# ucla-vision/xivo

Measured on AMD Instinct MI355X. Metric: EKF updates/sec (state dim 250, 80 feats) @1 GPU; % MFMA roofline, higher is better.
Workload: dtype f64; 1 GPU; MH gating + UpdateJosephForm: state dim 250, 80 features (M=160), XIVO row sparsity, P/H/inn/R resident in HBM; filters_per_gpu=16384, global_batch=16384, parallelism=replicas x1 (no collective), pipeline=sparse-H (row-pair compressed H, whitened in-solve Joseph form), hand_over=dense H -> row-pair compressed rows every step, inside the timed region, route=sparse_in_solve, not_spd_filters=0

## Files before the change

### xivo_amd/csrc/capi_update.hip

```cpp
#include <algorithm>

#include "capi_internal.h"

using namespace xivo_hip;
using namespace xivo_hip::capi;

namespace {

enum UpdateRoute : int { ROUTE_FUSED = 0, ROUTE_SPARSE_IN_SOLVE, ROUTE_SPARSE_WHITENED, ROUTE_SPARSE_SYMMETRIC, ROUTE_SPARSE_TAIL,
                         ROUTE_DENSE_ASCODED, ROUTE_DENSE_WHITENED, ROUTE_DENSE_SYMMETRIC, ROUTE_COUNT };
static const char* kRouteNames[ROUTE_COUNT] = {"fused", "sparse_in_solve", "sparse_whitened", "sparse_symmetric", "sparse_tail",
                                               "dense_ascoded", "dense_whitened", "dense_symmetric"};
struct UpdatePlan {
  int route;
  bool sparse;
  bool in_solve;
  bool latency;
  bool stream8;
  bool f32_whitened;
};

static UpdatePlan plan_update(const xivo_hip_ctx* c, int b0, int B, bool gate) {
  const StagedRows& r = c->rows;
  const int Np = c->Np, Mp = r.rows_padded();
// ... 106 lines not shown
    StageTimer st(c, ST_TRSM, (2.0 * Mf * Mf * Nf + 32.0 * Mf * Nf + (plan.in_solve ? 2.0 * t_outs_f * Mf : 0.0)) * B, label,
                  8.0 * B * (0.5 * Mp * (Mp + 1) + Mp / 16 * 512.0 + (plan.in_solve ? 1.0 : 3.0) * Np * Mp + (plan.in_solve ? t_outs + (double)Np * Np : 0.0)));
    HIP_TRY((hipError_t)(narrow ? launch_trsm_narrow(a, c->stream) : launch_trsm_f64(a, c->stream)));
    if (plan.in_solve) return XIVO_HIP_OK;
  }
  GemmExtra x; x.epi = EPI_RSUB_MAT; x.msub = v.P; x.lower_only = 1; x.skip = v.status;
  x.small_tiles = plan.latency;
  if (plan.f32_whitened) {
    x.fp32 = 1; x.a_f32 = 1; x.b_f32 = 1;
    const WhitenedF32 w = whitened_f32(v.G, Np, Mp);
    return gemm(c, ST_PNEW, B, Np, Np, {w.V, w.Y, Mp}, v.P, x);
  }
  return gemm(c, ST_PNEW, B, Np, Np, {v.K, v.G, Mp}, v.P, x);
}

static int update_sparse_range(xivo_hip_ctx* c, const UpdatePlan& plan, const UpdateViews& v, int b0, int B, const UpdateGate* gate) {
  const int Np = c->Np, Mp = c->rows.rows_padded();
  const BatchMat &P = v.P, &HP = v.HP, &PHT = v.PHT, &S = v.S, &K = v.K, &G = v.G, &T = v.T;
  const BatchVec &inn = v.inn, &diagR = v.diagR;
  const EllBuffers& e = v.ell;
  const auto [nc_max, pw_max] = c->rows.max_slots(b0, B);
  const double Nf = c->N, Mf = c->rows.rows();
  const double nnz_flops = 2.0 * Mf * 21.0;
  int rc;
  if (plan.route == ROUTE_FUSED) {
    FusedArgs a{};
    P.to(a.P, a.strideP, a.ldp); a.ell = e; inn.to(a.inn, a.strideInn); diagR.to(a.diagR, a.strideR);
    v.err.to(a.err, a.strideErr); PHT.to(a.PHT, a.stridePHT, a.ldpht); a.status = v.status;
    a.Np = Np; a.Mp = Mp; a.batch = B; a.pw = pw_max;
    if (gate) {
      a.gate = 1; a.F = gate->F; a.gp = gate->gp;
      a.mask = c->mask + (long)b0 * gate->F; a.dist = c->dist + (long)b0 * gate->F;
      if (c->rows.dense_alive()) { v.H.to(a.H, a.strideH, a.ldh); v.HT.to(a.HT, a.strideHT, a.ldht); }
    }
    char label[64]; fused_update_label(Mp, Np, pw_max, label, sizeof(label));
    const double t_outs_f = 0.5 * Nf * (Nf + 1.0);
    StageTimer st(c, ST_TRSM, (nnz_flops * (Nf + Mf) + Mf * Mf * Mf / 3.0 + 2.0 * Mf * Mf * Nf + 32.0 * Mf * Nf + 2.0 * t_outs_f * Mf) * B, label,
                  B * (16.0 * Np * Np + (Mp / 2) * ELL_W * 20.0));
    HIP_TRY((hipError_t)launch_fused_update(a, c->stream));
    return XIVO_HIP_OK;
  }
  const int mr0 = c->rows.mixed_row0();
  const int Mp_ell = mr0 >= 0 ? round_up16(mr0) : Mp;
  const int oos_pad = mr0 >= 0 ? round_up16(Mp - mr0) : 0;
  bool walk_tiled = false;
  const int oos_k = (mr0 >= 0 && c->have_layout) ? std::min(Np, round_up16(c->lay.group_begin + 6 * c->lay.n_groups)) : Np;
  {
    EllMulArgs a{}; a.ell = e; P.to(a.Src, a.strideSrc, a.ldsrc); PHT.to(a.out, a.strideOut, a.ldo);
    HP.to(a.out2, a.strideOut2, a.ldo2); a.X = Np; a.Mp = Mp_ell; a.batch = B; a.nc_max = nc_max; a.pw_max = pw_max; a.cols = Np;
    char label[64]; ell_kernel_label(ELL_HP, a, label, sizeof(label));
    walk_tiled = ell_uses_slab_form(a);
    StageTimer st(c, ST_HP, nnz_flops * Nf * B, label, 8.0 * B * ((double)Np * Np + (double)Np * Mp));
    HIP_TRY((hipError_t)launch_ell_mul(ELL_HP, a, c->stream));
  }
  if (mr0 >= 0) {
    GemmExtra x; x.C2 = PHT.at(0, mr0);
    rc = gemm(c, ST_HP, B, oos_pad, Np, {v.H.at(mr0, 0), P, oos_k}, HP.at(mr0, 0), x);
    if (rc) return rc;
  }
  const bool lead = c->rows.has_lead() && mr0 < 0;
  if (lead) {
    GemmExtra x; x.epi = EPI_ADD_MAT; x.msub = PHT; x.C2 = HP;
    x.c2_rows = walk_tiled ? LEAD_K : 0;
    rc = gemm(c, ST_HP, B, Np, Mp, {P, v.lead, LEAD_K}, PHT, x);
    if (rc) return rc;
  }
  GateEllArgs ga{};
  if (gate) {
    ga.ell = e;
    v.H.to(ga.H, ga.strideH, ga.ldh); v.HT.to(ga.HT, ga.strideHT, ga.ldht);
    if (!c->rows.dense_alive()) { ga.H = nullptr; ga.HT = nullptr; }
    ga.PHT = PHT.p;
    inn.to(ga.inn, ga.strideInn); diagR.to(ga.diagR, ga.strideR);
    ga.mask = c->mask + (long)b0 * gate->F; ga.dist = c->dist + (long)b0 * gate->F;
    ga.F = gate->F; ga.Np = Np; ga.batch = B;
    S.to(ga.S, ga.strideS, ga.lds); ga.Mp = Mp; ga.gp = gate->gp;
  }
  const BatchVec Sdiag{T.p, T.stride};
  int diag_done = 0;
  {
    EllMulArgs a{}; a.ell = e; PHT.to(a.Src, a.strideSrc, a.ldsrc); HP.to(a.SrcAlt, a.strideSrcAlt, a.ldsrcAlt);
    S.to(a.out, a.strideOut, a.ldo); a.cols = Np;
    diagR.to(a.diagR, a.strideR); a.X = Mp; a.Mp = Mp_ell; a.batch = B; a.nc_max = nc_max; a.pw_max = pw_max;
    if (gate && mr0 < 0 && !lead && (long)2 * Mp <= Sdiag.stride) { Sdiag.to(a.diag_out, a.strideDiag); a.diag_done = &diag_done; }
    char label[64]; ell_kernel_label(ELL_S, a, label, sizeof(label));
    StageTimer st(c, ST_S, nnz_flops * Mf * B, label, 8.0 * B * ((double)Np * Mp + (double)Mp * Mp));
    HIP_TRY((hipError_t)launch_ell_mul(ELL_S, a, c->stream));
  }
  if (mr0 >= 0) {
    GemmExtra x; x.epi = EPI_ADD_DIAG; x.diag = BatchVec{diagR.p + mr0, diagR.stride}; x.lower_only = 1;
    rc = gemm(c, ST_S, B, oos_pad, oos_pad, {HP.at(mr0, 0), v.H.at(mr0, 0), oos_k}, S.at(mr0, mr0), x);
    if (rc) return rc;
  }
  if (lead) {
    GemmExtra x; x.epi = EPI_ADD_MAT; x.msub = S; x.lower_only = 1;
    rc = gemm(c, ST_S, B, Mp, Mp, {HP, v.lead, LEAD_K}, S, x);
    if (rc) return rc;
  }
  CholGateArgs cg{};
  bool gate_folded = false;
  if (gate) {
    if (diag_done) Sdiag.to(ga.Sdiag, ga.strideSdiag);
    gate_folded = diag_done && !c->rows.dense_alive() && mr0 < 0 && !plan.latency && chol_gate_supported(Mp, B);
    if (gate_folded) {
      Sdiag.to(cg.Sdiag, cg.strideSdiag); inn.to(cg.inn, cg.strideInn); diagR.to(cg.diagR, cg.strideR);
      cg.ellval = e.val; cg.strideVal = e.stride_val(); cg.ell_w = ELL_W; PHT.to(cg.PHT, cg.stridePHT, cg.ldpht); cg.Np = Np;
      cg.mask = ga.mask; cg.dist = ga.dist; cg.F = gate->F; cg.gp = gate->gp;
    } else {
      StageTimer st(c, ST_GATE, 0.0, "gate_ell_kernel");
      HIP_TRY((hipError_t)launch_gate_ell(ga, c->stream));
    }
  }
  if (plan.route != ROUTE_SPARSE_TAIL && plan.route != ROUTE_SPARSE_SYMMETRIC)
    return finish_whitened(c, plan, v, B, gate_folded ? &cg : nullptr);
  rc = factor_S(c, v, B, 0, gate_folded ? &cg : nullptr, Mf * Mf * Mf / 3.0 * B);
  if (rc) return rc;
  if (plan.route == ROUTE_SPARSE_SYMMETRIC) return finish_symmetric(c, plan, v, B);
  const bool t_here = trsm_forms_T(Mp, Np);
  {
    TrsmArgs a = trsm_args(c, v, B);
    if (t_here) { T.to(a.T, a.strideT, a.ldt); P.to(a.Pm, a.stridePm, a.ldpm); }
    char label[64]; trsm_kernel_label(Mp, label, sizeof(label), t_here ? 1 : 0);
    const double t_outs = 0.5 * Np * (Np + 1.0), t_outs_f = 0.5 * Nf * (Nf + 1.0);
    StageTimer st(c, ST_TRSM, (2.0 * Mf * Mf * Nf + (t_here ? 2.0 * t_outs_f * Mf : 0.0)) * B, label,
                  8.0 * B * (0.5 * Mp * (Mp + 1) + Mp / 16 * 512.0 + 2.0 * Np * Mp + (t_here ? t_outs + (double)Np * Np : 0.0)));
    HIP_TRY((hipError_t)launch_trsm_f64(a, c->stream));
  }
  if (!t_here) {
    GemmExtra x; x.epi = EPI_SUB_MAT; x.msub = P; x.lower_only = 1;
    rc = gemm(c, ST_AP, B, Np, Np, {K, PHT, Mp}, T, x);
    if (rc) return rc;
  }
  {
    EllMulArgs a{}; a.ell = e; T.to(a.Src, a.strideSrc, a.ldsrc); G.to(a.out, a.strideOut, a.ldo);
    diagR.to(a.diagR, a.strideR); K.to(a.K, a.strideK, a.ldk); a.X = Np; a.Mp = Mp; a.batch = B; a.nc_max = nc_max; a.pw_max = pw_max; a.cols = Np;
    char label[64]; ell_kernel_label(ELL_G, a, label, sizeof(label));
    StageTimer st(c, ST_KH, nnz_flops * Np * B, label, 8.0 * B * ((double)Np * Np + 2.0 * Np * Mp));
    HIP_TRY((hipError_t)launch_ell_mul(ELL_G, a, c->stream));
  }
  if (pnew_reg_supported(Mp, Np)) {
    PnewRegArgs a{}; G.to(a.G, a.strideG, a.ldg); K.to(a.K, a.strideK, a.ldk);
    T.to(a.T, a.strideT, a.ldt); P.to(a.P, a.strideP, a.ldp);
    a.skip_status = v.status; a.Mp = Mp; a.Np = Np; a.batch = B;
    char label[64]; pnew_reg_kernel_label(Mp, label, sizeof(label));
    const double outs = 0.5 * Np * (Np + 1.0);
    StageTimer st(c, ST_PNEW, 2.0 * outs * Mp * B, label, 8.0 * B * (2.0 * Np * Mp + outs + (double)Np * Np));
    HIP_TRY((hipError_t)launch_pnew_reg_f64(a, c->stream));
    return XIVO_HIP_OK;
  }
  GemmExtra x; x.epi = EPI_SUB_MAT; x.msub = T; x.lower_only = 1;
  x.skip = v.status;
  return gemm(c, ST_PNEW, B, Np, Np, {G, K, Mp}, P, x);
}

static int update_dense_range(xivo_hip_ctx* c, const UpdatePlan& plan, const UpdateViews& v, int b0, int B, const UpdateGate* gate) {
  const int Np = c->Np, Mp = c->rows.rows_padded();
  const BatchMat &H = v.H, &HT = v.HT, &P = v.P, &HP = v.HP, &PHT = v.PHT, &S = v.S, &K = v.K, &A = v.KHI, &T = v.T;
  int rc = ensure_dense(c);
  if (rc) return rc;
  {
    GemmExtra x; x.C2 = PHT;
    rc = gemm(c, ST_HP, B, Mp, Np, {H, P, Np}, HP, x);
    if (rc) return rc;
  }
  if (gate) {
    rc = ensure_HT(c);
    if (rc) return rc;
    GateDenseArgs a{};
    H.to(a.Hw, a.strideH, a.ldh); HT.to(a.HTw, a.strideHT, a.ldht);
// ... 417 lines not shown
```

### xivo_amd/csrc/ell.h

```cpp
#pragma once
#include "common.h"

namespace xivo_hip {

constexpr int ELL_CW = 16, ELL_PW = 12, ELL_W = ELL_CW + ELL_PW;
constexpr int ELL_PIW = 12;

struct EllBuffers {
  int* idx;
  double* val;
  int* nc;
  int* pw;
  int* over;
  int pairs_max;
  __host__ __device__ long stride_idx() const { return (long)pairs_max * ELL_W; }
  __host__ __device__ long stride_val() const { return (long)pairs_max * ELL_W * 2; }
};

int launch_meas_compress(const double* H, long strideH, int ldh, const double* inn, long strideInn,
                         const double* diagR, long strideR, int M, int N, int Np, int Mp_clear, EllBuffers e,
                         double* inn_out, long strideInnOut, double* R_out, long strideROut, int batch, hipStream_t s,
                         int* host_flags = nullptr );
bool meas_compress_fits(int Mp_clear, int Np);
int launch_meas_vectors(const double* inn, long strideInn, const double* diagR, long strideR, int M, int Mp_clear, EllBuffers e,
                        double* inn_out, long strideInnOut, double* R_out, long strideROut, int batch, hipStream_t s);
int launch_ell_to_dense(EllBuffers e, double* H, long strideH, int ldh, double* HT, long strideHT, int ldht, int Mp,
                        int Np, int batch, hipStream_t s, int Mrows = -1);
int launch_zero_rows(double* H, long strideH, int ldh, int row0, int nrows, int c0, int c1, int batch, hipStream_t s);

enum EllMode : int {
  ELL_HP = 0,
  ELL_S = 1,
  ELL_G = 2,
  ELL_GF = 3,
};
struct GateEllArgs {
  EllBuffers ell;
  double* H; long strideH; int ldh;
  double* HT; long strideHT; int ldht;
  double* PHT;
  double* inn; long strideInn;
  double* diagR; long strideR;
  unsigned char* mask; double* dist;
  int F, Np, batch;
  GateParams gp;
  double* S; long strideS; int lds; int Mp;
  const double* Sdiag; long strideSdiag;
};
struct EllMulArgs {
  EllBuffers ell;
  const double* Src; long strideSrc; int ldsrc;
  int cols;
  const double* SrcAlt; long strideSrcAlt; int ldsrcAlt;
  double* out; long strideOut; int ldo;
  double* out2; long strideOut2; int ldo2;
  double* diag_out; long strideDiag;
  int* diag_done;
  const double* diagR; long strideR;
  const double* K; long strideK; int ldk;
  int X;
  int Mp;
  int slabs_per_wg;
  int persist_stride;
  int rb_per_wg;
  int nc_max;
  int pw_max;
  int batch;
};
int launch_ell_mul(int mode, const EllMulArgs& a, hipStream_t s);
void ell_kernel_label(int mode, const EllMulArgs& a, char* buf, size_t n);
bool ell_uses_slab_form(const EllMulArgs& a);

int launch_gate_ell(const GateEllArgs& a, hipStream_t s);

}
```

### xivo_amd/csrc/ell_kernels.hip

```cpp
#include "ell.h"
#include <stdio.h>
#include <stdlib.h>

namespace xivo_hip {

namespace {

struct MeasCompressArgs {
  const double* H; long strideH; int ldh;
  const double* inn; long strideInn;
  const double* diagR; long strideR;
  int M, N, Np;
  int pairs_clear;
  EllBuffers ell;
  double* inn_out; long strideInnOut;
  double* R_out; long strideROut;
  int list_ld;
  int* host_flags;
};

template <bool ALIGNED, int UNR = 16>
__global__ __launch_bounds__(256) void meas_compress_kernel(MeasCompressArgs a) {
  extern __shared__ __attribute__((aligned(16))) double csh[];
  const int filt = blockIdx.x, tid = threadIdx.x, lane = tid & 63, wave = tid >> 6, nw = blockDim.x >> 6;
// ... 152 lines not shown
__global__ __launch_bounds__(256) void zero_rows_kernel(double* Hall, long strideH, int ldh, int row0, int nrows, int c0, int c1) {
  double* H = Hall + (long)blockIdx.x * strideH;
  for (long i = threadIdx.x; i < (long)nrows * (c1 - c0); i += 256) H[row0 + (i % nrows) + (long)(c0 + i / nrows) * ldh] = 0.0;
}

template <int MODE, int CWU>
__global__ __launch_bounds__(256) void ell_mul_kernel(EllMulArgs a) {
  const int xchunks = (a.X + 255) / 256;
  const int nrb = a.Mp / 16;
  const int rsplit = (nrb + a.rb_per_wg - 1) / a.rb_per_wg;
  const int per = rsplit * xchunks;
  const int b = blockIdx.x;
  const int xcd = b & 7, slot = b >> 3;
  const int filt = (slot / per) * 8 + xcd;
  if (filt >= a.batch) return;
  const int sub = slot % per;
  const int rs = sub / xchunks, xc = sub % xchunks;
  const int x = xc * 256 + threadIdx.x;
  const bool live = x < a.X;
  const int xs = live ? x : 0;
  const double* __restrict__ Src = a.Src + (long)filt * a.strideSrc + xs;
  const int* __restrict__ idx0 = a.ell.idx + (long)filt * a.ell.stride_idx();
  const double* __restrict__ val0 = a.ell.val + (long)filt * a.ell.stride_val();

  double cm[CWU];
#pragma unroll
  for (int t = 0; t < CWU; ++t) cm[t] = Src[(long)idx0[t] * a.ldsrc];

  const double* __restrict__ dR = a.diagR + (long)filt * a.strideR;
  const double* __restrict__ K = a.K + (long)filt * a.strideK + xs;
  double* __restrict__ out = a.out + (long)filt * a.strideOut + xs;
  double* __restrict__ out2 = a.out2 + (long)filt * a.strideOut2 + (long)xs * a.ldo2;
  const int p_end = 8 * min(nrb, (rs + 1) * a.rb_per_wg);
#pragma unroll 2
  for (int p = 8 * rs * a.rb_per_wg; p < p_end; ++p) {
    const int* __restrict__ pi = idx0 + (long)p * ELL_W + ELL_CW;
    const double* __restrict__ pv = val0 + (long)p * ELL_W * 2;
    double sv[ELL_PW];
#pragma unroll
    for (int t = 0; t < ELL_PW; ++t) sv[t] = Src[(long)pi[t] * a.ldsrc];
    double a0 = 0.0, a1 = 0.0;
#pragma unroll
    for (int t = 0; t < CWU; ++t) { a0 = fma(pv[2 * t], cm[t], a0); a1 = fma(pv[2 * t + 1], cm[t], a1); }
#pragma unroll
    for (int t = 0; t < ELL_PW; ++t) {
      a0 = fma(pv[2 * (ELL_CW + t)], sv[t], a0); a1 = fma(pv[2 * (ELL_CW + t) + 1], sv[t], a1);
    }
    if (!live) continue;
    const int m = 2 * p;
    if (MODE == ELL_HP) {
      out[(long)m * a.ldo] = a0;
      out[(long)(m + 1) * a.ldo] = a1;
      *reinterpret_cast<d2*>(out2 + m) = d2{a0, a1};
    } else if (MODE == ELL_S) {
      out[(long)m * a.ldo] = a0 + (x == m ? dR[m] : 0.0);
      out[(long)(m + 1) * a.ldo] = a1 + (x == m + 1 ? dR[m + 1] : 0.0);
    } else {
      out[(long)m * a.ldo] = fma(K[(long)m * a.ldk], dR[m], a0);
      out[(long)(m + 1) * a.ldo] = fma(K[(long)(m + 1) * a.ldk], dR[m + 1], a1);
    }
  }
}

typedef __attribute__((address_space(4))) const double ell_cdouble;
typedef __attribute__((address_space(4))) const int ell_cint;

constexpr bool ell_tile_pf(int mode, int cwu, int xc, int pwu) {
  return xc == 64 && cwu == 12 && mode == ELL_S && pwu >= 0;
}
typedef unsigned ell_u2 __attribute__((ext_vector_type(2)));
__device__ __forceinline__ __amdgpu_buffer_rsrc_t ell_rsrc(const void* p) {
  return __builtin_amdgcn_make_buffer_rsrc(const_cast<void*>(p), 0, 0x7FFFFFFF, 0x00020000);
}
__device__ __forceinline__ double ell_buf_ld(__amdgpu_buffer_rsrc_t r, unsigned voff, unsigned soff) {
  return __builtin_bit_cast(double, __builtin_amdgcn_raw_buffer_load_b64(r, voff, soff, 0));
}
__device__ __forceinline__ void ell_buf_st(double v, __amdgpu_buffer_rsrc_t r, unsigned voff, unsigned soff) {
  __builtin_amdgcn_raw_buffer_store_b64(__builtin_bit_cast(ell_u2, v), r, voff, soff, 0);
}

constexpr bool ell_tile_mf(int mode, int cwu, int xc, int pwu) {
  return (xc == 64 || xc == 32) && cwu % 4 == 0 && pwu % 3 == 0 && (mode == ELL_HP || mode == ELL_S);
}
constexpr int ell_tile_threads(int mode, int cwu, int xc, int pwu) {
  return (mode == ELL_S || ell_tile_pf(mode, cwu, xc, pwu)) ? 512 : 1024;
}

template <int MODE, int CWU, int XC, int PWU, bool TALL = true>
__global__ __launch_bounds__(ell_tile_threads(MODE, CWU, XC, PWU)) void ell_tile_kernel(EllMulArgs a) {
  constexpr int NSLOT = CWU + PWU;
  constexpr int NT = ell_tile_threads(MODE, CWU, XC, PWU), NW = NT / 64;
  constexpr bool PF = ell_tile_pf(MODE, CWU, XC, PWU);
  constexpr int UNR = (PF || (CWU == 12 && XC == 64)) ? 2 : 1;
  constexpr int RN = PF ? (MODE == ELL_S ? (TALL ? 40 : 32) : 34) : 8;
  extern __shared__ __attribute__((aligned(16))) double tile[];
  const int xchunks = (a.X + XC - 1) / XC;
  const int wgs = (xchunks + a.slabs_per_wg - 1) / a.slabs_per_wg;
  const int b = blockIdx.x;
  const int xcd = b & 7, slot = b >> 3;
  int filt = (slot / wgs) * 8 + xcd;
  if (filt >= a.batch) return;
  const int s_begin = (slot % wgs) * a.slabs_per_wg;
  const int s_end = min(xchunks, s_begin + a.slabs_per_wg);
  const int tid = threadIdx.x, lane = tid & 63, wave = __builtin_amdgcn_readfirstlane(tid >> 6);
  const double* Src = a.Src + (long)filt * a.strideSrc;
  const int cols = a.cols;
  const int pairs = a.Mp / 2;
  double* ops = tile + (long)cols * XC;
  unsigned short* pidx = reinterpret_cast<unsigned short*>(ops + (long)pairs * NSLOT * 2);
  auto stage_ops = [&](int f) {
    const d2* __restrict__ gv = reinterpret_cast<const d2*>(a.ell.val + (long)f * a.ell.stride_val());
    for (int e = tid; e < pairs * NSLOT; e += NT) {
      const int p = e / NSLOT, t = e % NSLOT;
      *reinterpret_cast<d2*>(ops + 2 * e) = gv[p * ELL_W + (t < CWU ? t : ELL_CW + (t - CWU))];
    }
    const int* __restrict__ gi = a.ell.idx + (long)f * a.ell.stride_idx();
    for (int e = tid; e < pairs * ELL_PIW; e += NT) {
      const int p = e / ELL_PIW, t = e % ELL_PIW;
      pidx[e] = t < PWU ? (unsigned short)gi[p * ELL_W + ELL_CW + t] : (unsigned short)0;
    }
    if (tid < ELL_CW) pidx[pairs * ELL_PIW + tid] = (unsigned short)gi[tid];
  };
  stage_ops(filt);
  double r[RN];
  auto fetch = [&](const double* FSrc, int sidx) {
    const int x0 = sidx * XC;
    if (MODE == ELL_S) {
      constexpr int KU = RN / (XC / NW);
      const __amdgpu_buffer_rsrc_t rs = ell_rsrc(FSrc);
      const unsigned vo = (unsigned)lane * 8u;
#pragma unroll
      for (int q = 0; q < XC / NW; ++q) {
        const int jj = wave + NW * q;
        const bool ok = x0 + jj < a.X;
        const unsigned so = (unsigned)((x0 + (ok ? jj : 0)) * a.ldsrc) * 8u;
#pragma unroll
        for (int u = 0; u < KU; ++u) {
          const int k = lane + 64 * u;
          r[q * KU + u] = (ok && k < cols) ? ell_buf_ld(rs, vo, so + (unsigned)(64 * u) * 8u) : 0.0;
        }
      }
    } else {
      const int xx = tid % XC, kq = tid / XC;
      const bool ok = x0 + xx < a.X;
      const unsigned voff = ((unsigned)(ok ? xx : 0) + (unsigned)kq * (unsigned)a.ldsrc) * 8u;
      const char* base = reinterpret_cast<const char*>(FSrc + x0);
      const size_t step = (size_t)(NT / XC) * (size_t)a.ldsrc * 8u;
      const int nu = cols / (NT / XC);
#pragma unroll
      for (int u = 0; u < RN; ++u) {
        double v = 0.0;
        if (u < nu) v = *reinterpret_cast<const double*>(base + (size_t)u * step + voff);
        r[u] = ok ? v : 0.0;
      }
    }
  };
  auto park = [&]() {
    if (MODE == ELL_S) {
      constexpr int KU = RN / (XC / NW);
#pragma unroll
      for (int q = 0; q < XC / NW; ++q) {
        const int jj = wave + NW * q;
#pragma unroll
        for (int u = 0; u < KU; ++u) { const int k = lane + 64 * u; if (k < cols) tile[k * XC + (jj ^ (k & 15))] = r[q * KU + u]; }
      }
    } else {
      const int xx = tid % XC, kq = tid / XC;
#pragma unroll
      for (int u = 0; u < RN; ++u) { const int k = kq + (NT / XC) * u; if (k < cols) tile[k * XC + (xx ^ (k & 15))] = r[u]; }
    }
  };

  const int xx = lane % XC, half = lane / XC;
  auto slab = [&](int k) -> double { return tile[k * XC + (xx ^ (k & 15))]; };

  const int fstep = PF ? a.persist_stride : 0;
  if (PF) fetch(Src, s_begin);
  for (;;) {
  ell_cint* idx0 = (ell_cint*)(a.ell.idx + (long)filt * a.ell.stride_idx());
  ell_cdouble* dR = (ell_cdouble*)(a.diagR + (long)filt * a.strideR);
  const int nfilt = filt + fstep;
  const bool more = fstep > 0 && nfilt < a.batch;
  for (int sidx = s_begin; sidx < s_end; ++sidx) {
    if (PF) {
      park();
    } else if (MODE == ELL_S) {
      const int x0 = sidx * XC;
      for (int jj = wave; jj < XC; jj += NW) {
        const bool ok = x0 + jj < a.X;
        const double* __restrict__ col = Src + (long)(x0 + (ok ? jj : 0)) * a.ldsrc;
        for (int k0 = 0; k0 < cols; k0 += 64 * 8) {
#pragma unroll
          for (int u = 0; u < 8; ++u) { const int k = k0 + lane + 64 * u; r[u] = (ok && k < cols) ? col[k] : 0.0; }
#pragma unroll
          for (int u = 0; u < 8; ++u) { const int k = k0 + lane + 64 * u; if (k < cols) tile[k * XC + (jj ^ (k & 15))] = r[u]; }
        }
      }
    } else {
      const int x0 = sidx * XC;
      const int xq = tid % XC, kq = tid / XC;
      const bool ok = x0 + xq < a.X;
      const double* __restrict__ row = Src + x0 + (ok ? xq : 0);
      for (int k0 = 0; k0 < cols; k0 += (NT / XC) * 8) {
#pragma unroll
        for (int u = 0; u < 8; ++u) { const int k = k0 + kq + (NT / XC) * u; r[u] = (ok && k < cols) ? row[(long)k * a.ldsrc] : 0.0; }
#pragma unroll
        for (int u = 0; u < 8; ++u) { const int k = k0 + kq + (NT / XC) * u; if (k < cols) tile[k * XC + (xq ^ (k & 15))] = r[u]; }
      }
    }
    if (PF) asm volatile("s_waitcnt lgkmcnt(0)\n\ts_barrier" ::: "memory");
    else __syncthreads();
    if (PF) {
      if (sidx + 1 < s_end) fetch(Src, sidx + 1);
      else if (more) fetch(a.Src + (long)nfilt * a.strideSrc, s_begin);
    }

    if constexpr (ell_tile_mf(MODE, CWU, XC, PWU)) {
      constexpr int NC = XC / 16, KS = CWU / 4;
      const int li = lane & 15, lg = lane >> 4;
      const unsigned short* cidx = pidx + pairs * ELL_PIW;
      int ck[KS];
#pragma unroll
      for (int s = 0; s < KS; ++s) ck[s] = cidx[4 * s + lg];
      const int x0 = sidx * XC;
      const __amdgpu_buffer_rsrc_t rO = ell_rsrc(a.out + (long)filt * a.strideOut);
      const unsigned vO = (unsigned)(2 * lg * a.ldo + li) * 8u;
      double dRc[NC];
#pragma unroll
      for (int c = 0; c < NC; ++c) dRc[c] = 0.0;
      if (MODE == ELL_S) {
#pragma unroll
        for (int c = 0; c < NC; ++c) if (x0 + 16 * c + li < a.X) dRc[c] = a.diagR[(long)filt * a.strideR + x0 + 16 * c + li];
      }
      const int rb_end = MODE == ELL_S ? min(pairs / 8, NC * (sidx + 1)) : pairs / 8;
      const int pa = (li & 3) + 4 * (li >> 3), ra = (li >> 2) & 1;
      for (int rb = wave; rb < rb_end; rb += NW) {
        const int p0 = 8 * rb;
        d4 acc[NC];
#pragma unroll
        for (int c = 0; c < NC; ++c) acc[c] = d4{0.0, 0.0, 0.0, 0.0};
        if constexpr (NT == 512) {
          uint2 iq[2][ELL_PIW / 4];
  #pragma unroll
          for (int q = 0; q < 2; ++q) {
            const uint2* pq = reinterpret_cast<const uint2*>(pidx + (p0 + lg + 4 * q) * ELL_PIW);
  #pragma unroll
            for (int u = 0; u < ELL_PIW / 4; ++u) iq[q][u] = pq[u];
          }
  #pragma unroll
          for (int q = 0; q < 2; ++q) {
            const int p = p0 + lg + 4 * q;
            const d2* pv = reinterpret_cast<const d2*>(ops) + (long)p * NSLOT + CWU;
            static_assert(PWU % 3 == 0, "three slots per step");
            d2 vn[3];
  #pragma unroll
            for (int u = 0; u < 3; ++u) vn[u] = pv[u];
  #pragma unroll
            for (int t0 = 0; t0 < PWU; t0 += 3) {
              d2 v[3]; double g[3][NC];
  #pragma unroll
              for (int u = 0; u < 3; ++u) {
                const int t = t0 + u;
                v[u] = vn[u];
                const unsigned w = (t & 2) ? iq[q][t >> 2].y : iq[q][t >> 2].x;
                const int k = (int)((t & 1) ? (w >> 16) : (w & 0xffffu));
                const double* trow = tile + k * XC;
                const int sw = k & 15;
  #pragma unroll
                for (int c = 0; c < NC; ++c) g[u][c] = trow[(16 * c + li) ^ sw];
              }
              if (t0 + 3 < PWU) {
  #pragma unroll
                for (int u = 0; u < 3; ++u) vn[u] = pv[t0 + 3 + u];
              }
              __builtin_amdgcn_sched_barrier(0);
  #pragma unroll
              for (int u = 0; u < 3; ++u) {
  #pragma unroll
                for (int c = 0; c < NC; ++c) {
                  acc[c][2 * q] = fma(v[u][0], g[u][c], acc[c][2 * q]);
                  acc[c][2 * q + 1] = fma(v[u][1], g[u][c], acc[c][2 * q + 1]);
                }
              }
            }
          }
        } else {
  #pragma unroll
          for (int q = 0; q < 2; ++q) {
            const int p = p0 + lg + 4 * q;
            const d2* pv = reinterpret_cast<const d2*>(ops) + (long)p * NSLOT + CWU;
            const unsigned short* pkp = pidx + p * ELL_PIW;
            static_assert(PWU % 3 == 0, "three slots per step");
  #pragma unroll 1
            for (int t0 = 0; t0 < PWU; t0 += 3) {
              d2 v[3]; double g[3][NC];
  #pragma unroll
              for (int u = 0; u < 3; ++u) {
                v[u] = pv[t0 + u];
                const int k = (int)pkp[t0 + u];
                const double* trow = tile + k * XC;
                const int sw = k & 15;
  #pragma unroll
                for (int c = 0; c < NC; ++c) g[u][c] = trow[(16 * c + li) ^ sw];
              }
              __builtin_amdgcn_sched_barrier(0);
  #pragma unroll
              for (int u = 0; u < 3; ++u) {
  #pragma unroll
                for (int c = 0; c < NC; ++c) {
                  acc[c][2 * q] = fma(v[u][0], g[u][c], acc[c][2 * q]);
                  acc[c][2 * q + 1] = fma(v[u][1], g[u][c], acc[c][2 * q + 1]);
                }
              }
            }
          }
        }
        {
          double av[KS], cb[KS][NC];
#pragma unroll
          for (int s = 0; s < KS; ++s) {
            av[s] = ops[((long)(p0 + pa) * NSLOT + 4 * s + lg) * 2 + ra];
#pragma unroll
            for (int c = 0; c < NC; ++c) cb[s][c] = tile[ck[s] * XC + ((16 * c + li) ^ (ck[s] & 15))];
          }
#pragma unroll
          for (int c = 0; c < NC; ++c) {
#pragma unroll
            for (int s = 0; s < KS; ++s) acc[c] = __builtin_amdgcn_mfma_f64_16x16x4f64(av[s], cb[s][c], acc[c], 0, 0, 0);
          }
        }
#pragma unroll
        for (int c = 0; c < NC; ++c) {
          const int x = x0 + 16 * c + li;
          if (x >= a.X) continue;
#pragma unroll
          for (int r = 0; r < 4; ++r) {
            const int pp = p0 + lg + 4 * (r >> 1), i = r & 1, m = 2 * pp + i;
            const unsigned sO = (unsigned)((2 * p0 + 8 * (r >> 1) + i) * a.ldo + x0 + 16 * c) * 8u;
            if (MODE == ELL_HP) ell_buf_st(acc[c][r], rO, vO, sO);
            else {
              const double sv_ = acc[c][r] + (x == m ? dRc[c] : 0.0);
              ell_buf_st(sv_, rO, vO, sO);
              if (a.diag_out && (x >> 1) == pp) a.diag_out[(long)filt * a.strideDiag + 4 * pp + 2 * (x & 1) + i] = sv_;
            }
          }
        }
      }
      asm volatile("s_waitcnt lgkmcnt(0)\n\ts_barrier" ::: "memory");
      continue;
    }
    const int x = sidx * XC + xx;
    const bool live = x < a.X;
    const double* __restrict__ K = a.K + (long)filt * a.strideK + (live ? x : 0);
    double* __restrict__ out = a.out + (long)filt * a.strideOut + (live ? x : 0);
    float* __restrict__ outf = reinterpret_cast<float*>(a.out) + (long)filt * a.strideOut + (live ? x : 0);
    double cm[CWU];
#pragma unroll
    for (int t = 0; t < CWU; ++t) cm[t] = slab(idx0[t]);
    const int p_end = MODE == ELL_S ? min(pairs, (sidx * XC + XC) / 2) : pairs;
    double dRx = 0.0;
    if (MODE == ELL_S && live) dRx = a.diagR[(long)filt * a.strideR + x];
#pragma unroll UNR
    for (int p = wave; p < p_end; p += NW) {
      const d2* pv = reinterpret_cast<const d2*>(ops) + (long)p * NSLOT;
      unsigned pk[ELL_PIW];
      {
        const uint2* pq = reinterpret_cast<const uint2*>(pidx + p * ELL_PIW);
#pragma unroll
        for (int u = 0; u < ELL_PIW / 4; ++u) {
          const uint2 q = pq[u];
          pk[4 * u] = q.x & 0xffffu; pk[4 * u + 1] = q.x >> 16; pk[4 * u + 2] = q.y & 0xffffu; pk[4 * u + 3] = q.y >> 16;
        }
      }
      double sv[PWU];
#pragma unroll
      for (int t = 0; t < PWU; ++t) sv[t] = slab((int)pk[t]);
      double a0 = 0.0, a1 = 0.0;
#pragma unroll
      for (int t = 0; t < CWU; ++t) { const d2 v = pv[t]; a0 = fma(v[0], cm[t], a0); a1 = fma(v[1], cm[t], a1); }
#pragma unroll
      for (int t = 0; t < PWU; ++t) { const d2 v = pv[CWU + t]; a0 = fma(v[0], sv[t], a0); a1 = fma(v[1], sv[t], a1); }
      if (!live) continue;
#pragma unroll
      for (int i = 0; i < 2; ++i) {
        if (XC == 32 && i != half) continue;
        const int m = 2 * p + i;
        const double acc = i ? a1 : a0;
        if (MODE == ELL_HP) out[(long)m * a.ldo] = acc;
        else if (MODE == ELL_S) {
          const double sv_ = acc + (x == m ? dRx : 0.0);
          out[(long)m * a.ldo] = sv_;
          if (XC == 64 && a.diag_out && (x >> 1) == p) a.diag_out[(long)filt * a.strideDiag + 4 * p + 2 * (x & 1) + i] = sv_;
        }
        else if (MODE == ELL_GF) outf[(long)m * a.ldo] = (float)fma(K[(long)m * a.ldk], dR[m], acc);
        else out[(long)m * a.ldo] = fma(K[(long)m * a.ldk], dR[m], acc);
      }
    }
    asm volatile("s_waitcnt lgkmcnt(0)\n\ts_barrier" ::: "memory");
  }
  if (!more) break;
  stage_ops(nfilt);
  filt = nfilt;
  Src = a.Src + (long)filt * a.strideSrc;
  }
}

}

#define CHECK_LAUNCH() return (int)hipGetLastError()

int launch_meas_compress(const double* H, long strideH, int ldh, const double* inn, long strideInn,
                         const double* diagR, long strideR, int M, int N, int Np, int Mp_clear, EllBuffers e,
                         double* inn_out, long strideInnOut, double* R_out, long strideROut, int batch, hipStream_t s,
                         int* host_flags) {
  if (batch <= 0) return 0;
  MeasCompressArgs a;
  a.host_flags = host_flags;
  a.H = H; a.strideH = strideH; a.ldh = ldh; a.inn = inn; a.strideInn = strideInn; a.diagR = diagR; a.strideR = strideR;
  a.M = M; a.N = N; a.Np = Np; a.pairs_clear = Mp_clear / 2; a.ell = e;
  a.inn_out = inn_out; a.strideInnOut = strideInnOut; a.R_out = R_out; a.strideROut = strideROut;
  const int nt = ((a.pairs_clear + 63) / 64) * 64;
  if (nt > 256) return (int)hipErrorInvalidValue;
  a.list_ld = (a.pairs_clear + 3) & ~3;
  const size_t lds = (size_t)ELL_W * a.list_ld * (sizeof(d2) + sizeof(int)) + (size_t)(nt / 64 + 1) * Np * sizeof(int);
  const bool aligned = (ldh % 2 == 0) && (strideH % 2 == 0) && ((reinterpret_cast<uintptr_t>(H) & 15u) == 0) && (M % 2 == 0);
  static bool attr_set = false;
  if (!attr_set) {
    const int cap = 160 * 1024 - 256;
    hipError_t e1 = hipFuncSetAttribute(reinterpret_cast<const void*>(&meas_compress_kernel<true>), hipFuncAttributeMaxDynamicSharedMemorySize, cap);
// ... 3 lines not shown
  }
  if (lds > (size_t)(160 * 1024 - 256)) return (int)hipErrorInvalidValue;
  if (aligned) hipLaunchKernelGGL(meas_compress_kernel<true>, dim3(batch), dim3(nt), lds, s, a);
  else hipLaunchKernelGGL(meas_compress_kernel<false>, dim3(batch), dim3(nt), lds, s, a);
  CHECK_LAUNCH();
}

static size_t meas_compress_lds(int Mp_clear, int Np) {
  const int pairs_clear = Mp_clear / 2;
  const int nt = ((pairs_clear + 63) / 64) * 64;
  const int list_ld = (pairs_clear + 3) & ~3;
  return (size_t)ELL_W * list_ld * (sizeof(d2) + sizeof(int)) + (size_t)(nt / 64 + 1) * Np * sizeof(int);
}
bool meas_compress_fits(int Mp_clear, int Np) {
  return Mp_clear / 2 <= 256 && meas_compress_lds(Mp_clear, Np) <= (size_t)(160 * 1024 - 256);
}
int launch_meas_vectors(const double* inn, long strideInn, const double* diagR, long strideR, int M, int Mp_clear, EllBuffers e,
                        double* inn_out, long strideInnOut, double* R_out, long strideROut, int batch, hipStream_t s) {
  if (batch <= 0) return 0;
  hipLaunchKernelGGL(meas_vectors_kernel, dim3(batch), dim3(256), 0, s, inn, strideInn, diagR, strideR, M, Mp_clear, e, inn_out,
                     strideInnOut, R_out, strideROut);
  CHECK_LAUNCH();
}

int launch_ell_to_dense(EllBuffers e, double* H, long strideH, int ldh, double* HT, long strideHT, int ldht, int Mp,
                        int Np, int batch, hipStream_t s, int Mrows) {
  if (batch <= 0) return 0;
  hipLaunchKernelGGL(ell_to_dense_kernel, dim3(batch), dim3(256), 0, s, e, H, strideH, ldh, HT, strideHT, ldht, Mp, Np,
                     Mrows < 0 ? Mp : Mrows);
  CHECK_LAUNCH();
}
int launch_zero_rows(double* H, long strideH, int ldh, int row0, int nrows, int c0, int c1, int batch, hipStream_t s) {
  if (batch <= 0 || nrows <= 0 || c1 <= c0) return 0;
  hipLaunchKernelGGL(zero_rows_kernel, dim3(batch), dim3(256), 0, s, H, strideH, ldh, row0, nrows, c0, c1);
  CHECK_LAUNCH();
}

template <int MODE, int CWU, int XC, int PWU, bool TALL = true>
static int launch_ell_tile_t(const EllMulArgs& a_in, size_t lds, hipStream_t s) {
  if constexpr (TALL && MODE == ELL_S && ell_tile_pf(MODE, CWU, XC, PWU)) {
    if (a_in.cols <= 256) return launch_ell_tile_t<MODE, CWU, XC, PWU, false>(a_in, lds, s);
  }
  static bool attr_set = false;
  if (!attr_set) {
    (void)hipFuncSetAttribute(reinterpret_cast<const void*>(&ell_tile_kernel<MODE, CWU, XC, PWU, TALL>),
                              hipFuncAttributeMaxDynamicSharedMemorySize, 160 * 1024);
    attr_set = true;
  }
  EllMulArgs a = a_in;
  const int xchunks = (a.X + XC - 1) / XC;
  a.slabs_per_wg = ((ell_tile_pf(MODE, CWU, XC, PWU) || MODE == ELL_HP) && a.batch >= 1024) ? xchunks : 1;
  const int wgs = (xchunks + a.slabs_per_wg - 1) / a.slabs_per_wg;
  int grid = ((a.batch + 7) / 8) * 8 * wgs;
  a.persist_stride = 0;
  if (ell_tile_pf(MODE, CWU, XC, PWU) && wgs == 1) {
    static int cus = 0;
    if (!cus) { int dev = 0; (void)hipGetDevice(&dev); (void)hipDeviceGetAttribute(&cus, hipDeviceAttributeMultiprocessorCount, dev); if (cus < 8) cus = 8; }
    const int G = cus / 8 * 8;
    if (grid > 2 * G) { a.persist_stride = G; grid = G; }
  }
  if (!(MODE == ELL_S && XC == 64)) a.diag_out = nullptr;
  if (a_in.diag_done) *a_in.diag_done = a.diag_out ? 1 : 0;
  hipLaunchKernelGGL((ell_tile_kernel<MODE, CWU, XC, PWU, TALL>), dim3(grid), dim3(ell_tile_threads(MODE, CWU, XC, PWU)), lds, s, a);
  return (int)hipGetLastError();
}
static void ell_pick(const EllMulArgs& a, int* xc, int* cwu, int* pwu, size_t* lds) {
  *cwu = a.nc_max <= 12 ? 12 : ELL_CW;
  *pwu = (*cwu == 12 && a.pw_max > 0 && a.pw_max <= 9) ? 9 : ELL_PW;
  const size_t pidx = ((size_t)(a.Mp / 2) * ELL_PIW + ELL_CW) * sizeof(unsigned short);
  const size_t ops = (size_t)(a.Mp / 2) * (*cwu + *pwu) * 2 * sizeof(double) + pidx;
  const size_t lds64 = (size_t)a.cols * 64 * sizeof(double) + ops, lds32 = (size_t)a.cols * 32 * sizeof(double) + ops;
  const size_t cap = 160 * 1024;
  *xc = 0; *lds = 0;
  if (lds64 <= cap) { *xc = 64; *lds = lds64; return; }
  if (lds32 <= cap) { *xc = 32; *lds = lds32; }
}

bool ell_uses_slab_form(const EllMulArgs& a) {
  int xc, cwu, pwu; size_t lds;
  ell_pick(a, &xc, &cwu, &pwu, &lds);
  return xc != 0;
}

void ell_kernel_label(int mode, const EllMulArgs& a, char* buf, size_t n) {
  int xc, cwu, pwu; size_t lds;
  ell_pick(a, &xc, &cwu, &pwu, &lds);
  if (xc) snprintf(buf, n, "ell_tile_kernel<%d,%d,%d,%d>", mode, cwu, xc, pwu);
  else snprintf(buf, n, "ell_mul_kernel<%d,%d>", mode, cwu);
}

template <int MODE>
static int launch_ell_tile_m(const EllMulArgs& a, hipStream_t s, bool* done) {
  int xc, cwu, pwu; size_t lds;
  ell_pick(a, &xc, &cwu, &pwu, &lds);
  *done = xc != 0;
  const bool n12 = cwu == 12;
  if (xc == 64 && pwu == 9) return launch_ell_tile_t<MODE, 12, 64, 9>(a, lds, s);
  if (xc == 64) return n12 ? launch_ell_tile_t<MODE, 12, 64, ELL_PW>(a, lds, s) : launch_ell_tile_t<MODE, ELL_CW, 64, ELL_PW>(a, lds, s);
  if (xc == 32 && pwu == 9) return launch_ell_tile_t<MODE, 12, 32, 9>(a, lds, s);
  if (xc == 32) return n12 ? launch_ell_tile_t<MODE, 12, 32, ELL_PW>(a, lds, s) : launch_ell_tile_t<MODE, ELL_CW, 32, ELL_PW>(a, lds, s);
  return 0;
}

int launch_ell_mul(int mode, const EllMulArgs& a_in, hipStream_t s) {
  if (a_in.batch <= 0) return 0;
  if (a_in.diag_done) *a_in.diag_done = 0;
  EllMulArgs a = a_in;
  {
    {
      bool done = false;
      const int rc = mode == ELL_HP ? launch_ell_tile_m<ELL_HP>(a, s, &done)
                     : (mode == ELL_S ? launch_ell_tile_m<ELL_S>(a, s, &done)
                     : (mode == ELL_GF ? launch_ell_tile_m<ELL_GF>(a, s, &done) : launch_ell_tile_m<ELL_G>(a, s, &done)));
      if (done) return rc;
    }
  }
  if (mode == ELL_S) {
    a.Src = a.SrcAlt; a.strideSrc = a.strideSrcAlt; a.ldsrc = a.ldsrcAlt;
  }
  const int xchunks = (a.X + 255) / 256;
  const int nrb = a.Mp / 16;
  a.rb_per_wg = (long)a.batch * xchunks >= 2048 ? nrb : ((long)a.batch * xchunks >= 512 ? (nrb + 1) / 2 : 1);
  const int rsplit = (nrb + a.rb_per_wg - 1) / a.rb_per_wg;
  const int grid = ((a.batch + 7) / 8) * 8 * rsplit * xchunks;
#define ELL_LAUNCH(MODE)                                                                                  \
  do {                                                                                                    \
    if (a.nc_max <= 12) hipLaunchKernelGGL((ell_mul_kernel<MODE, 12>), dim3(grid), dim3(256), 0, s, a);   \
    else hipLaunchKernelGGL((ell_mul_kernel<MODE, ELL_CW>), dim3(grid), dim3(256), 0, s, a);              \
  } while (0)
  switch (mode) {
    case ELL_HP: ELL_LAUNCH(ELL_HP); break;
    case ELL_S: ELL_LAUNCH(ELL_S); break;
    default: ELL_LAUNCH(ELL_G); break;
  }
#undef ELL_LAUNCH
  CHECK_LAUNCH();
}

}
```

Measured before the change: 987,200 updates/s.

## Skip strictly-upper S tiles and balance lower-triangle tiles across waves in ELL_S

The ELL_S tile kernel now works on 16-column sub-tiles and skips those strictly above the diagonal when no lead GEMM needs the upper part, since S is consumed lower-only. The remaining lower-triangle tiles are spread evenly across waves in variable-width chunks, instead of each wave taking whole row blocks. The prefetch of the next slab is folded into the LDS park step, and diagR values are prefetched once per slab and broadcast with shuffles. The bandwidth model in the stage timer is updated to match. Risks are extra dispatch branching, smaller MFMA chunks, and possible reads of the upper part by consumers not covered by keep_upper.

```diff
diff --git a/xivo_amd/csrc/capi_update.hip b/xivo_amd/csrc/capi_update.hip
--- a/xivo_amd/csrc/capi_update.hip
+++ b/xivo_amd/csrc/capi_update.hip
@@ -212,9 +212,10 @@
     EllMulArgs a{}; a.ell = e; PHT.to(a.Src, a.strideSrc, a.ldsrc); HP.to(a.SrcAlt, a.strideSrcAlt, a.ldsrcAlt);
     S.to(a.out, a.strideOut, a.ldo); a.cols = Np;
     diagR.to(a.diagR, a.strideR); a.X = Mp; a.Mp = Mp_ell; a.batch = B; a.nc_max = nc_max; a.pw_max = pw_max;
+    a.keep_upper = lead ? 1 : 0;
     if (gate && mr0 < 0 && !lead && (long)2 * Mp <= Sdiag.stride) { Sdiag.to(a.diag_out, a.strideDiag); a.diag_done = &diag_done; }
     char label[64]; ell_kernel_label(ELL_S, a, label, sizeof(label));
-    StageTimer st(c, ST_S, nnz_flops * Mf * B, label, 8.0 * B * ((double)Np * Mp + (double)Mp * Mp));
+    StageTimer st(c, ST_S, nnz_flops * Mf * B, label, B * (8.0 * Np * Mp + ell_s_bytes_written(a)));
     HIP_TRY((hipError_t)launch_ell_mul(ELL_S, a, c->stream));
   }
   if (mr0 >= 0) {
diff --git a/xivo_amd/csrc/ell.h b/xivo_amd/csrc/ell.h
--- a/xivo_amd/csrc/ell.h
+++ b/xivo_amd/csrc/ell.h
@@ -62,6 +62,7 @@
   int Mp;
   int slabs_per_wg;
   int persist_stride;
+  int keep_upper;
   int rb_per_wg;
   int nc_max;
   int pw_max;
@@ -70,6 +71,7 @@
 int launch_ell_mul(int mode, const EllMulArgs& a, hipStream_t s);
 void ell_kernel_label(int mode, const EllMulArgs& a, char* buf, size_t n);
 bool ell_uses_slab_form(const EllMulArgs& a);
+double ell_s_bytes_written(const EllMulArgs& a);
 
 int launch_gate_ell(const GateEllArgs& a, hipStream_t s);
 
diff --git a/xivo_amd/csrc/ell_kernels.hip b/xivo_amd/csrc/ell_kernels.hip
--- a/xivo_amd/csrc/ell_kernels.hip
+++ b/xivo_amd/csrc/ell_kernels.hip
@@ -258,6 +258,7 @@
 constexpr bool ell_tile_mf(int mode, int cwu, int xc, int pwu) {
   return (xc == 64 || xc == 32) && cwu % 4 == 0 && pwu % 3 == 0 && (mode == ELL_HP || mode == ELL_S);
 }
+template <int V> struct ell_ic { static constexpr int value = V; };
 constexpr int ell_tile_threads(int mode, int cwu, int xc, int pwu) {
   return (mode == ELL_S || ell_tile_pf(mode, cwu, xc, pwu)) ? 512 : 1024;
 }
@@ -331,14 +332,24 @@
       }
     }
   };
-  auto park = [&]() {
+  static_assert(!PF || MODE == ELL_S, "the prefetching form is the S instantiation");
+  auto park = [&](const double* FSrc, int nsidx, bool have) {
     if (MODE == ELL_S) {
       constexpr int KU = RN / (XC / NW);
+      const __amdgpu_buffer_rsrc_t rs = ell_rsrc(FSrc);
+      const unsigned vo = (unsigned)lane * 8u;
+      const int nx0 = nsidx * XC;
 #pragma unroll
       for (int q = 0; q < XC / NW; ++q) {
         const int jj = wave + NW * q;
-#pragma unroll
-        for (int u = 0; u < KU; ++u) { const int k = lane + 64 * u; if (k < cols) tile[k * XC + (jj ^ (k & 15))] = r[q * KU + u]; }
+        const bool ok = have && nx0 + jj < a.X;
+        const unsigned so = (unsigned)((nx0 + (ok ? jj : 0)) * a.ldsrc) * 8u;
+#pragma unroll
+        for (int u = 0; u < KU; ++u) {
+          const int k = lane + 64 * u;
+          if (k < cols) tile[k * XC + (jj ^ (k & 15))] = r[q * KU + u];
+          r[q * KU + u] = (ok && k < cols) ? ell_buf_ld(rs, vo, so + (unsigned)(64 * u) * 8u) : 0.0;
+        }
       }
     } else {
       const int xx = tid % XC, kq = tid / XC;
@@ -350,6 +361,13 @@
   const int xx = lane % XC, half = lane / XC;
   auto slab = [&](int k) -> double { return tile[k * XC + (xx ^ (k & 15))]; };
 
+  constexpr bool SMF = MODE == ELL_S && ell_tile_mf(MODE, CWU, XC, PWU);
+  auto load_dR = [&](int f, int s) -> double {
+    const int xr = s * XC + lane % XC;
+    return xr < a.X ? a.diagR[(long)f * a.strideR + xr] : 0.0;
+  };
+  double dRn = 0.0;
+  if (SMF) dRn = load_dR(filt, s_begin);
   const int fstep = PF ? a.persist_stride : 0;
   if (PF) fetch(Src, s_begin);
   for (;;) {
@@ -358,8 +376,11 @@
   const int nfilt = filt + fstep;
   const bool more = fstep > 0 && nfilt < a.batch;
   for (int sidx = s_begin; sidx < s_end; ++sidx) {
+    const double dRs = dRn;
+    const bool last = sidx + 1 == s_end, have = !last || more;
+    const int nf = last && more ? nfilt : filt, ns = last ? s_begin : sidx + 1;
     if (PF) {
-      park();
+      park(a.Src + (long)nf * a.strideSrc, ns, have);
     } else if (MODE == ELL_S) {
       const int x0 = sidx * XC;
       for (int jj = wave; jj < XC; jj += NW) {
@@ -386,11 +407,8 @@
     }
     if (PF) asm volatile("s_waitcnt lgkmcnt(0)\n\ts_barrier" ::: "memory");
     else __syncthreads();
-    if (PF) {
-      if (sidx + 1 < s_end) fetch(Src, sidx + 1);
-      else if (more) fetch(a.Src + (long)nfilt * a.strideSrc, s_begin);
-    }
-
+
+    if (SMF && have) dRn = load_dR(nf, ns);
     if constexpr (ell_tile_mf(MODE, CWU, XC, PWU)) {
       constexpr int NC = XC / 16, KS = CWU / 4;
       const int li = lane & 15, lg = lane >> 4;
@@ -401,20 +419,19 @@
       const int x0 = sidx * XC;
       const __amdgpu_buffer_rsrc_t rO = ell_rsrc(a.out + (long)filt * a.strideOut);
       const unsigned vO = (unsigned)(2 * lg * a.ldo + li) * 8u;
-      double dRc[NC];
-#pragma unroll
-      for (int c = 0; c < NC; ++c) dRc[c] = 0.0;
-      if (MODE == ELL_S) {
-#pragma unroll
-        for (int c = 0; c < NC; ++c) if (x0 + 16 * c + li < a.X) dRc[c] = a.diagR[(long)filt * a.strideR + x0 + 16 * c + li];
-      }
       const int rb_end = MODE == ELL_S ? min(pairs / 8, NC * (sidx + 1)) : pairs / 8;
       const int pa = (li & 3) + 4 * (li >> 3), ra = (li >> 2) & 1;
-      for (int rb = wave; rb < rb_end; rb += NW) {
-        const int p0 = 8 * rb;
-        d4 acc[NC];
-#pragma unroll
-        for (int c = 0; c < NC; ++c) acc[c] = d4{0.0, 0.0, 0.0, 0.0};
+      auto step = [&](auto nb_tag, int rb, int c0) {
+        constexpr int NB = decltype(nb_tag)::value;
+        const int p0 = 8 * rb, cofs = 16 * c0;
+        double dRv = 0.0;
+        if (MODE == ELL_S) {
+          const int cd = rb - NC * sidx;
+          if (cd >= c0 && cd < c0 + NB) dRv = __shfl(dRs, 16 * cd + li);
+        }
+        d4 acc[NB];
+#pragma unroll
+        for (int c = 0; c < NB; ++c) acc[c] = d4{0.0, 0.0, 0.0, 0.0};
         if constexpr (NT == 512) {
           uint2 iq[2][ELL_PIW / 4];
   #pragma unroll
@@ -433,17 +450,17 @@
             for (int u = 0; u < 3; ++u) vn[u] = pv[u];
   #pragma unroll
             for (int t0 = 0; t0 < PWU; t0 += 3) {
-              d2 v[3]; double g[3][NC];
+              d2 v[3]; double g[3][NB];
   #pragma unroll
               for (int u = 0; u < 3; ++u) {
                 const int t = t0 + u;
                 v[u] = vn[u];
                 const unsigned w = (t & 2) ? iq[q][t >> 2].y : iq[q][t >> 2].x;
                 const int k = (int)((t & 1) ? (w >> 16) : (w & 0xffffu));
-                const double* trow = tile + k * XC;
+                const double* trow = tile + k * XC + cofs;
                 const int sw = k & 15;
   #pragma unroll
-                for (int c = 0; c < NC; ++c) g[u][c] = trow[(16 * c + li) ^ sw];
+                for (int c = 0; c < NB; ++c) g[u][c] = trow[(16 * c + li) ^ sw];
               }
               if (t0 + 3 < PWU) {
   #pragma unroll
@@ -453,7 +470,7 @@
   #pragma unroll
               for (int u = 0; u < 3; ++u) {
   #pragma unroll
-                for (int c = 0; c < NC; ++c) {
+                for (int c = 0; c < NB; ++c) {
                   acc[c][2 * q] = fma(v[u][0], g[u][c], acc[c][2 * q]);
                   acc[c][2 * q + 1] = fma(v[u][1], g[u][c], acc[c][2 * q + 1]);
                 }
@@ -469,21 +486,21 @@
             static_assert(PWU % 3 == 0, "three slots per step");
   #pragma unroll 1
             for (int t0 = 0; t0 < PWU; t0 += 3) {
-              d2 v[3]; double g[3][NC];
+              d2 v[3]; double g[3][NB];
   #pragma unroll
               for (int u = 0; u < 3; ++u) {
                 v[u] = pv[t0 + u];
                 const int k = (int)pkp[t0 + u];
-                const double* trow = tile + k * XC;
+                const double* trow = tile + k * XC + cofs;
                 const int sw = k & 15;
   #pragma unroll
-                for (int c = 0; c < NC; ++c) g[u][c] = trow[(16 * c + li) ^ sw];
+                for (int c = 0; c < NB; ++c) g[u][c] = trow[(16 * c + li) ^ sw];
               }
               __builtin_amdgcn_sched_barrier(0);
   #pragma unroll
               for (int u = 0; u < 3; ++u) {
   #pragma unroll
-                for (int c = 0; c < NC; ++c) {
+                for (int c = 0; c < NB; ++c) {
                   acc[c][2 * q] = fma(v[u][0], g[u][c], acc[c][2 * q]);
                   acc[c][2 * q + 1] = fma(v[u][1], g[u][c], acc[c][2 * q + 1]);
                 }
@@ -492,35 +509,65 @@
           }
         }
         {
-          double av[KS], cb[KS][NC];
+          double av[KS], cb[KS][NB];
 #pragma unroll
           for (int s = 0; s < KS; ++s) {
             av[s] = ops[((long)(p0 + pa) * NSLOT + 4 * s + lg) * 2 + ra];
 #pragma unroll
-            for (int c = 0; c < NC; ++c) cb[s][c] = tile[ck[s] * XC + ((16 * c + li) ^ (ck[s] & 15))];
+            for (int c = 0; c < NB; ++c) cb[s][c] = tile[ck[s] * XC + cofs + ((16 * c + li) ^ (ck[s] & 15))];
           }
 #pragma unroll
-          for (int c = 0; c < NC; ++c) {
+          for (int c = 0; c < NB; ++c) {
 #pragma unroll
             for (int s = 0; s < KS; ++s) acc[c] = __builtin_amdgcn_mfma_f64_16x16x4f64(av[s], cb[s][c], acc[c], 0, 0, 0);
           }
         }
 #pragma unroll
-        for (int c = 0; c < NC; ++c) {
-          const int x = x0 + 16 * c + li;
+        for (int c = 0; c < NB; ++c) {
+          const int x = x0 + cofs + 16 * c + li;
           if (x >= a.X) continue;
 #pragma unroll
           for (int r = 0; r < 4; ++r) {
             const int pp = p0 + lg + 4 * (r >> 1), i = r & 1, m = 2 * pp + i;
-            const unsigned sO = (unsigned)((2 * p0 + 8 * (r >> 1) + i) * a.ldo + x0 + 16 * c) * 8u;
+            const unsigned sO = (unsigned)((2 * p0 + 8 * (r >> 1) + i) * a.ldo + x0 + cofs + 16 * c) * 8u;
             if (MODE == ELL_HP) ell_buf_st(acc[c][r], rO, vO, sO);
             else {
-              const double sv_ = acc[c][r] + (x == m ? dRc[c] : 0.0);
+              const double sv_ = acc[c][r] + (x == m ? dRv : 0.0);
               ell_buf_st(sv_, rO, vO, sO);
               if (a.diag_out && (x >> 1) == pp) a.diag_out[(long)filt * a.strideDiag + 4 * pp + 2 * (x & 1) + i] = sv_;
             }
           }
         }
+      };
+      if constexpr (MODE == ELL_S) {
+        const int chi = min(NC, (a.X - x0 + 15) / 16);
+        const int nfull = a.keep_upper ? rb_end : min(rb_end, NC * sidx), nd = min(rb_end - nfull, chi);
+        const int total = nfull * chi + nd * chi - nd * (nd - 1) / 2;
+        const int cap = (total + NW - 1) / NW;
+        int pos = wave * cap;
+        const int hi = min(total, pos + cap);
+        if (pos < hi) {
+          int rb, c;
+          if (pos < nfull * chi) { rb = pos / chi; c = pos - rb * chi; }
+          else {
+            int q = pos - nfull * chi, d = 0;
+            while (q >= chi - d) { q -= chi - d; ++d; }
+            rb = nfull + d; c = d + q;
+          }
+          while (pos < hi) {
+            const int n = min(chi - c, hi - pos);
+            if (n == 1) step(ell_ic<1>{}, rb, c);
+            else if (n == 2) step(ell_ic<2>{}, rb, c);
+            else if constexpr (NC > 2) {
+              if (n == 3) step(ell_ic<3>{}, rb, c);
+              else step(ell_ic<NC>{}, rb, c);
+            }
+            pos += n; c += n;
+            if (c == chi) { ++rb; c = rb < nfull ? 0 : rb - NC * sidx; }
+          }
+        }
+      } else {
+        for (int rb = wave; rb < rb_end; rb += NW) step(ell_ic<NC>{}, rb, 0);
       }
       asm volatile("s_waitcnt lgkmcnt(0)\n\ts_barrier" ::: "memory");
       continue;
@@ -690,6 +737,20 @@
   return xc != 0;
 }
 
+double ell_s_bytes_written(const EllMulArgs& a) {
+  int xc, cwu, pwu; size_t lds;
+  ell_pick(a, &xc, &cwu, &pwu, &lds);
+  if (!xc) return 8.0 * a.X * a.Mp;
+  const int NC = xc / 16;
+  long tiles = 0;
+  for (int sidx = 0; sidx * xc < a.X; ++sidx) {
+    const int rb_end = std::min(a.Mp / 16, NC * (sidx + 1)), chi = std::min(NC, (a.X - sidx * xc + 15) / 16);
+    const int nfull = a.keep_upper ? rb_end : std::min(rb_end, NC * sidx), nd = std::min(rb_end - nfull, chi);
+    tiles += nfull * chi + nd * chi - nd * (nd - 1) / 2;
+  }
+  return 2048.0 * tiles;
+}
+
 void ell_kernel_label(int mode, const EllMulArgs& a, char* buf, size_t n) {
   int xc, cwu, pwu; size_t lds;
   ell_pick(a, &xc, &cwu, &pwu, &lds);
```

After: 1.001 million updates/s, median of 6. 1.01x the previous value.
